# mnhrk15/integrated_path_planning

Measured on AMD Instinct MI355X. Metric: candidate trajectories/sec, higher is better.
Workload: dtype f64; 1 GPU; config4: 256 ego instances/GPU x 2240-candidate lattice (5 s, dt 0.1 s), 20-sample x 30-pedestrian x 51-step fp32 prediction distribution (layout [S][P][T][2]), eps=0; 8 distinct batches rotated (501 MB of obstacle tensors per GPU); instances_per_gpu=256, instances_total=256, rotation_batches=8, plan_calls_in_flight=4

## Files before the change

### integrated_path_planning_amd/csrc/fot_host.cpp

```cpp
#include <hip/hip_runtime.h>

#include <algorithm>
#include <cmath>
#include <cstddef>
#include <cstdlib>
#include <atomic>
#include <chrono>
#include <cstring>
#include <mutex>
#include <new>
#include <string>
#include <thread>
#include <unordered_set>
#include <vector>

#include "fot_kernels.h"
#include "fot_math.hpp"
#include "fot_replay.hpp"
#include "fot_summary.hpp"
#include "fot_loopscore.hpp"
#include "fot_setup.hpp"
#include "fot_sgan.h"

using namespace fot;
// ... 209 lines not shown
struct Scenario {
    fot_params params = fot_params();
    DevParams P;
    HostSpline spline;
    DevBuf dSpline;
    bool has_path = false;
    TileShapes shapes;
    int32_t shape_base = 0;
};

constexpr int FOT_LANES = 4;
constexpr int FOT_SPLIT_MIN_INSTANCES = 32;

struct fot_handle {
    int device = 0;
    hipStream_t stream = nullptr;
    hipEvent_t fork = nullptr;
    hipEvent_t order_done = nullptr;
    hipStream_t order_stream = nullptr;
    bool order_valid = false;
    int eval_segments = 0;
    PinnedBuf hDone;
    int32_t done_seq = 0;
    bool done_seq_armed = false;
    int tile_cut = 0;
    int eval_form = 0;
    int last_eval_forms = 0;
    std::vector<Scenario> sc;
    std::vector<ScenarioRef> refs;
    DevBuf dP;
    DevBuf dSplineTab;
    int32_t n_shape_entries = 0;
    DevBuf dShapes;
    Workspace ws[FOT_LANES];
    int lanes_cfg = 1;
    int lanes_used = 0;
    DevBuf dUserStatic, dUserDyn, dOut;
    PinnedBuf hSmallIn, hSmallOut;
    PinnedBuf hRecOut;
    PinnedBuf hScoreIn, hScoreOut;
    DevBuf dScoreT;
    DevBuf dTmpA, dTmpB, dTmpC, dTmpD;
    LoopState loop;
    struct Sgan {
        bool loaded = false;
        fot_sgan_desc desc{};
        SgDev dev{};
        DevBuf dImg, dOff, dScene, dObs, dNoise, dOut, dHenc, dPool, dCtx, dH, dC, dXY;
        PinnedBuf hTab;
        void release()
        {
            for (DevBuf *b : { &dImg, &dOff, &dScene, &dObs, &dNoise, &dOut, &dHenc, &dPool, &dCtx, &dH, &dC, &dXY }) b->release();
            hTab.release();
        }
    } sgan;
    bool last_valid = false;
    bool prof_on = false;
    std::vector<hipEvent_t> prof_pool;
    size_t prof_used = 0;
    std::vector<int> prof_kernel;
    int32_t prof_launches[FOT_PROFILE_KERNELS] = { 0 };
    double prof_ms[FOT_PROFILE_KERNELS] = { 0 };
    std::string err;
};

namespace {
// ... 96 lines not shown
int upload_params(fot_handle *h)
{
    std::vector<DevParams> tab(h->sc.size());
    for (size_t s = 0; s < h->sc.size(); ++s) tab[s] = h->sc[s].P;
    HIP_TRY(h, hipSetDevice(h->device));
    HIP_TRY(h, hipDeviceSynchronize());
    HIP_TRY(h, h->dP.ensure(sizeof(DevParams) * tab.size()));
    HIP_TRY(h, hipMemcpy(h->dP.p, tab.data(), sizeof(DevParams) * tab.size(), hipMemcpyHostToDevice));
    h->last_valid = false;
    return FOT_OK;
}

int upload_tile_shapes(fot_handle *h, int cut)
{
    const size_t n_sc = h->sc.size();
    std::vector<const DevParams *> ps(n_sc);
    std::vector<TileShapes> shapes(n_sc);
    for (size_t s = 0; s < n_sc; ++s) ps[s] = &h->sc[s].P;
    build_tile_shapes(ps.data(), (int)n_sc, shapes.data(), cut);
    std::vector<int32_t> cand0, nn, span;
    for (size_t s = 0; s < n_sc; ++s) {
        h->sc[s].shape_base = (int32_t)cand0.size();
        cand0.insert(cand0.end(), shapes[s].cand0.begin(), shapes[s].cand0.end());
        nn.insert(nn.end(), shapes[s].n.begin(), shapes[s].n.end());
        span.insert(span.end(), shapes[s].span.begin(), shapes[s].span.end());
        h->sc[s].shapes = std::move(shapes[s]);
    }
    h->refs.assign(n_sc, ScenarioRef());
    for (size_t s = 0; s < n_sc; ++s) {
        h->refs[s].hp = &h->sc[s].params; h->refs[s].P = &h->sc[s].P;
        h->refs[s].shapes = &h->sc[s].shapes; h->refs[s].shape_base = h->sc[s].shape_base;
    }
    h->tile_cut = cut;
    const size_t nt = cand0.size();
    h->n_shape_entries = (int32_t)nt;
    HIP_TRY(h, hipSetDevice(h->device));
    HIP_TRY(h, hipDeviceSynchronize());
    HIP_TRY(h, h->dShapes.ensure(sizeof(int32_t) * 3 * std::max<size_t>(nt, 1)));
    if (nt) {
        HIP_TRY(h, hipMemcpy(h->dShapes.p, cand0.data(), sizeof(int32_t) * nt, hipMemcpyHostToDevice));
        HIP_TRY(h, hipMemcpy(h->dShapes.as<int32_t>() + nt, nn.data(), sizeof(int32_t) * nt, hipMemcpyHostToDevice));
        HIP_TRY(h, hipMemcpy(h->dShapes.as<int32_t>() + 2 * nt, span.data(), sizeof(int32_t) * nt, hipMemcpyHostToDevice));
    }
    h->last_valid = false;
    return FOT_OK;
}

int check_scenarios(fot_handle *h, const fot_batch &b, const int32_t *scen)
{
    const int n_inst = b.n_inst;
    if (!scen) return h->sc[0].has_path ? FOT_OK : fail(h, FOT_ERR_NO_PATH_SET, "fot_set_path_* has not been called");
    for (int i = 0; i < n_inst; ++i) {
        if (scen[i] < 0 || scen[i] >= (int)h->sc.size()) return fail(h, FOT_ERR_INVALID, "unknown scenario id");
        if (!h->sc[(size_t)scen[i]].has_path)
            return fail(h, FOT_ERR_NO_PATH_SET, "an instance's scenario has no path (fot_set_scenario_path_*)");
    }
    for (int i = 1; i < n_inst && b.ego; ++i)
        if (b.ego[i].has_prev_s == FOT_PREV_S_CHAINED && scen[i] != scen[i - 1])
            return fail(h, FOT_ERR_INVALID, "a chained instance must be on its predecessor's scenario (a chain is one planner)");
    return FOT_OK;
    return FOT_OK;
}

PathSet path_set(const fot_handle *h, const BatchLayout &L, const DevParams **P_launch)
{
    const DevParams *dP = h->dP.as<DevParams>();
    if (L.scens.size() <= 1) {
        const int s = L.scens.empty() ? 0 : L.scens[0];
        *P_launch = dP + s;
        return PathSet::single(spline_view(h, s));
    }
    PathSet ps;
    ps.table = h->dSplineTab.as<SplineView>();
    ps.mixed = 1;
    for (int s : L.scens) ps.knots[ps.n_knots++] = h->sc[(size_t)s].spline.n;
// ... 65 lines not shown
    const size_t slots = (size_t)std::max<int64_t>(L.n_slots, 1);
    HIP_TRY(h, w.dCost.ensure(sizeof(double) * slots));
    HIP_TRY(h, w.dParts.ensure(sizeof(TilePart) * (size_t)std::max(L.n_tiles, 1)));
    HIP_TRY(h, w.dStatus.ensure(slots));
    HIP_TRY(h, w.dKeep.ensure(sizeof(uint16_t) * slots));
    const size_t n_ent = (size_t)L.n_entries + 64;
    HIP_TRY(h, w.dEntCnt.ensure(sizeof(int32_t) * (size_t)P.n_total * (size_t)L.n_inst));
    HIP_TRY(h, w.dEnt32.ensure(sizeof(f2) * n_ent));
    HIP_TRY(h, w.dEnt64.ensure(sizeof(d2) * n_ent));
    HIP_TRY(h, w.dEntSid.ensure(n_ent));
    HIP_TRY(h, w.dWaveRng.ensure(sizeof(TileStep) * (size_t)P.n_total * (size_t)std::max(L.n_tiles, 1)));
    HIP_TRY(h, w.dNanFlag.ensure((size_t)std::max<int64_t>(L.n_tracks, 16)));
    HIP_TRY(h, w.dDone.ensure(sizeof(int32_t) * (size_t)L.n_inst));

    w.staging_pending[slot] = true;

    const InstDesc *d_desc = (const InstDesc *)w.dMeta.p;
    TileTable tt;
    tt.cand0 = h->dShapes.as<int32_t>();
    tt.n = h->dShapes.as<int32_t>() + h->n_shape_entries;
    tt.span = h->dShapes.as<int32_t>() + 2 * (size_t)h->n_shape_entries;
    tt.n_tiles = L.n_tiles; tt.max_tiles = L.max_tiles; tt.row_budget = L.row_budget;
    tt.eval_segments = h->eval_segments;
    tt.grouped = L.grouped;
    tt.lean = h->eval_form == 0 ? 1 : 0;
    for (const Scenario &S : h->sc) if (S.P.n_total > WAVE || S.P.has_footprint) tt.lean = 0;
    for (int i = 0; i < L.n_inst && tt.lean; ++i) if (L.desc[(size_t)i].max_viol != 0) tt.lean = 0;
    h->last_eval_forms |= tt.lean ? 2 : 1;
    GroupHeadOut gh;
    if (evaluate_in_groups(tt)) {
        gh.n_pos = L.max_tiles / GROUP_TILES;
        HIP_TRY(h, w.dHeads.ensure(sizeof(GroupHead) * (size_t)L.n_inst * (size_t)gh.n_pos));
        gh.heads = tt.heads = w.dHeads.as<GroupHead>();
        gh.tile_cand0 = tt.cand0; gh.tile_n = tt.n;
    }
    const DevParams *dP = nullptr;
    const PathSet sv = path_set(h, L, &dP);
    CandArrays ca;
    ca.cost = w.dCost.as<double>(); ca.parts = w.dParts.as<TilePart>();
    ca.status = w.dStatus.as<uint8_t>(); ca.keep = w.dKeep.as<uint16_t>();
    if (sync_caller && h->done_seq_armed) { ca.done_flag = (int32_t *)h->hDone.p; ca.done_seq = h->done_seq; }

    EntryArrays ea;
    ea.cnt = w.dEntCnt.as<int32_t>(); ea.e32 = w.dEnt32.as<f2>(); ea.e64 = w.dEnt64.as<d2>();
    ea.sid = w.dEntSid.as<uint8_t>(); ea.rng = w.dWaveRng.as<TileStep>();
    ea.nan_flag = w.dNanFlag.as<uint8_t>();
    MetaImport imp;
    imp.h_desc = (const InstDesc *)stg;
    imp.d_desc = (InstDesc *)w.dMeta.p;
    static const bool eager_env = getenv("FOT_NAN_SCAN") && !std::strcmp(getenv("FOT_NAN_SCAN"), "eager");
    const bool eager_nan = eager_env || d_dyn_stage != nullptr;
    ea.eager_nan = eager_nan ? 1 : 0;
    NanScan scan;
    scan.eager = ea.eager_nan;
    if (L.n_tracks > 0 && (L.any_tmajor || eager_nan)) {
        scan.dyn_xy = d_dyn; scan.dtype = b.obstacle_dtype; scan.flag = w.dNanFlag.as<uint8_t>();
        scan.blocks_per_inst = (int)std::min<int64_t>(64, std::max<int64_t>(1, (L.max_dyn_bytes + 262143) / 262144));
        if (d_dyn_stage) {
            scan.stage = d_dyn_stage; d_dyn = d_dyn_stage;
            scan.blocks_per_inst = (int)std::min<int64_t>(64, std::max<int64_t>(1, (L.max_dyn_bytes + 65535) / 65536));
        }
    }
    {
        ProfScope ps(h, 0, st);
        LAUNCH_TRY(h, launch_frenet_state(dP, sv, d_desc, w.dState.as<InstState>(), L.n_inst, imp, scan, w.dDone.as<int32_t>(), st, gh));
    }
    if (L.any_obstacles) {
// ... 206 lines not shown
    return (int32_t)live_handles().size();
}

void fot_destroy(fot_handle *h)
{
    if (!h) return;
    {
        std::lock_guard<std::mutex> lk(g_live_mu);
        auto &live = live_handles();
        auto it = live.find(h);
        if (it == live.end()) return;
        live.erase(it);
    }
    destroy_handle(h);
}

}

namespace {

void destroy_handle(fot_handle *h)
{
    const double budget = destroy_timeout_s();
    bool quiet = hipSetDevice(h->device) == hipSuccess;
    if (quiet && h->stream) quiet = drained([&] { return hipStreamQuery(h->stream); }, budget);
    if (quiet && h->order_valid) quiet = drained([&] { return hipEventQuery(h->order_done); }, budget);
    for (Workspace &w : h->ws) if (quiet && w.stream) quiet = drained([&] { return hipStreamQuery(w.stream); }, budget);
    if (!quiet) {
        (void)hipGetLastError();
        delete h;
        return;
    }
    for (Scenario &S : h->sc) S.dSpline.release();
    DevBuf *bufs[] = { &h->dP, &h->dSplineTab, &h->dShapes, &h->dUserStatic, &h->dUserDyn, &h->dOut, &h->dTmpA, &h->dTmpB, &h->dTmpC, &h->dTmpD
                     };
    for (DevBuf *b : bufs) b->release();
    for (Workspace &w : h->ws) w.release();
    h->hSmallIn.release(); h->hSmallOut.release(); h->hRecOut.release(); h->hDone.release();
    h->hScoreIn.release(); h->hScoreOut.release(); h->dScoreT.release();
    h->sgan.release();
    h->loop.release();
    for (hipEvent_t e : h->prof_pool) (void)hipEventDestroy(e);
    if (h->fork) (void)hipEventDestroy(h->fork);
    if (h->order_done) (void)hipEventDestroy(h->order_done);
    if (h->stream) (void)hipStreamDestroy(h->stream);
    delete h;
}

}

extern "C" {

int fot_set_scenario_path_waypoints(fot_handle *h, int32_t id, int32_t n, const double *wx, const double *wy)
{
    if (!h) return FOT_ERR_INVALID;
    if (id < 0 || id >= (int)h->sc.size()) return fail(h, FOT_ERR_INVALID, "unknown scenario id");
    std::string err;
    HostSpline sp;
    int rc = build_spline(n, wx, wy, sp, err);
    if (rc != FOT_OK) return fail(h, rc, err);
    h->sc[(size_t)id].spline = sp;
    return upload_spline(h, id);
}

int fot_set_path_waypoints(fot_handle *h, int32_t n, const double *wx, const double *wy)
{
    return fot_set_scenario_path_waypoints(h, 0, n, wx, wy);
// ... 2535 lines not shown
```

### integrated_path_planning_amd/csrc/fot_kernels.h

```cpp
#pragma once

#include <cstddef>
#include <hip/hip_runtime.h>
#include "fot_types.h"
#include "fot_summary.hpp"
#include "fot_predscore.hpp"
#include "fot_loopscore.hpp"
#include "fot_repsample.hpp"

namespace fot {

struct TilePart {
    double cost;
    int32_t idx, keep;
    int32_t cnt[8];
};

struct CandArrays {
    double *cost;
    uint8_t *status;
    uint16_t *keep;
    TilePart *parts;
    int32_t *done_flag = nullptr;
    int32_t done_seq = 0;
// ... 12 lines not shown
    uint8_t *sid;
    TileStep *rng;
    const uint8_t *nan_flag = nullptr;
    int eager_nan = 0;
};

struct NanScan {
    const void *dyn_xy = nullptr;
    int dtype = 0;
    uint8_t *flag = nullptr;
    int blocks_per_inst = 0;
    int eager = 0;
    void *stage = nullptr;
};

struct MetaImport {
    const InstDesc *h_desc = nullptr;
    InstDesc *d_desc = nullptr;
};

struct TileTable {
    const int32_t *cand0 = nullptr, *n = nullptr;
    const int32_t *span = nullptr;
    int n_tiles = 0, max_tiles = 0, row_budget = 0;
    int grouped = 0;
    int eval_segments = 0;
    int lean = 0;
    GroupHead *heads = nullptr;
};
bool evaluate_in_groups(const TileTable &tiles);

struct GroupHeadOut {
    GroupHead *heads = nullptr;
    const int32_t *tile_cand0 = nullptr, *tile_n = nullptr;
    int n_pos = 0;
};

struct PathSet {
    SplineView one = SplineView();
    const SplineView *table = nullptr;
    int mixed = 0;
    int n_knots = 0;
    int knots[FOT_MAX_SCENARIOS] = { 0 };
    int fit_knots(int cap) const
    {
        int m = 0;
        for (int i = 0; i < n_knots; ++i) if (knots[i] <= cap && knots[i] > m) m = knots[i];
        return m;
    }
    static PathSet single(const SplineView &sp)
    {
        PathSet ps;
        ps.one = sp; ps.n_knots = 1; ps.knots[0] = sp.n;
        return ps;
    }
};

int launch_frenet_state(const DevParams *P, const PathSet &ps, const InstDesc *desc, InstState *state, int n_inst,
                        MetaImport imp, NanScan scan, int32_t *inst_done, hipStream_t st,
                        GroupHeadOut gh = GroupHeadOut());
int launch_cull(const DevParams *P, const InstDesc *desc, const InstState *state, int n_inst, int n_total, int n_ext,
                const PathSet &ps, const void *static_xy, const void *dyn_xy, int dtype, EntryArrays e, TileTable tiles,
                hipStream_t st);
int launch_evaluate(const DevParams *P, const PathSet &ps, const InstDesc *desc, const InstState *state, int n_total,
                    int n_inst, TileTable tiles, EntryArrays e, CandArrays c, fot_result *out, int32_t *inst_done,
                    hipStream_t st);
int launch_debug_path(const DevParams *P, const InstDesc *desc, const InstState *state,
// ... 94 lines not shown
```

### integrated_path_planning_amd/csrc/fot_kernels.hip

```cpp
#include <hip/hip_runtime.h>

#include <cstdlib>

#include "fot_math.hpp"
#include "fot_kernels.h"
#include "fot_summary.hpp"
#include "fot_predscore.hpp"
#include "fot_loopscore.hpp"
#include "fot_repsample.hpp"

namespace fot {


template <int CTRL, int ROW_MASK>
__device__ __forceinline__ float dpp_f32(float v)
{
    return __int_as_float(__builtin_amdgcn_update_dpp(__float_as_int(v), __float_as_int(v), CTRL, ROW_MASK, 0xf, false));
}

#define FOT_WAVE_REDUCE_F32(NAME, OP)                                                        \
    __device__ __forceinline__ float NAME(float v)                                           \
    {                                                                                        \
        v = OP(v, dpp_f32<0xB1, 0xf>(v));                           \
        v = OP(v, dpp_f32<0x4E, 0xf>(v));                           \
// ... 259 lines not shown
            const bool at_upper = fabs(best_s - s_max) < 1e-3 && s_max < s_end;
            need_global = at_lower || at_upper;
        }
        if (need_global) {
            ScanBest b = block_argmin(scan_samples(sp, x, y, 0.0, s_end, n_glob, tid, FRENET_WG, true), s_best);
            best_s = linspace_at(0.0, s_end, n_glob, b.idx >= 0 ? b.idx : 0);
        }
        if (!given) best_s = refine_nearest_wave(sp, x, y, best_s, lane);
        const double new_prev_s = given ? NAN : best_s;

        double fr[6], ref[6];
        bool ok = given ? frenet_state_given(sp, D.ego, fr, ref) : frenet_state_at(sp, D.ego, best_s, fr, ref);
        if (!ok && !given) {
            double px, py;
            spline_xy(sp, best_s, px, py);
            if (isnan(px) || isnan(py)) {
                ScanBest b = block_argmin(scan_samples(sp, x, y, 0.0, s_end, n_glob, tid, FRENET_WG, true), s_best);
                best_s = linspace_at(0.0, s_end, n_glob, b.idx >= 0 ? b.idx : 0);
                ok = frenet_state_at(sp, D.ego, best_s, fr, ref);
            }
        }
        const int nb = (ok && fr[1] > 0.1) ? P.n_brake : 0;
        const int n_cand = ok ? D.n_grid + nb : 0;
        if (tid == 0) {
            if (inst_done) inst_done[inst] = 0;
            InstState &S = state[inst];
            for (int i = 0; i < 6; ++i) { S.frenet0[i] = ok ? fr[i] : NAN; S.ref0[i] = ok ? ref[i] : NAN; }
            S.new_prev_s = new_prev_s;
            S.c2f_ok = ok ? 1 : 0;
            S.n_brake = nb;
            S.n_cand = n_cand;
        }
        if (gh.heads) {
            for (int t = tid; t < gh.n_pos * GROUP_MAX_PROFILES; t += FRENET_WG) {
                const int pos = t / GROUP_MAX_PROFILES, p = t - pos * GROUP_MAX_PROFILES;
                GroupHead &H = gh.heads[(int64_t)inst * gh.n_pos + pos];
                GroupStage G;
                const int32_t kind = group_head_stage(P, D, fr, ok ? 1 : 0, n_cand, gh.tile_cand0, gh.tile_n, pos, G);
                if (kind != GROUP_HEAD_FULL) {
                    if (p == 0) group_head_none(kind, G, H);
                    continue;
                }
                if (p == 0) group_head_common(P, D, fr, G, H);
                if (p < GROUP_TILES) group_head_tile(P, D, fr, n_cand, gh.tile_cand0, gh.tile_n, G, p, H);
                group_head_profile(P, D, fr, G, p, H);
            }
        }
        carry_prev_s = new_prev_s;
        chained = true;
    }
}

__global__ void __launch_bounds__(FRENET_WG)
k_frenet_state(const DevParams *__restrict__ Pp, SplineView sp_hbm, const SplineView *__restrict__ sp_table, int mixed,
               int lds_knots, const InstDesc *desc, InstState *__restrict__ state, int n_inst, MetaImport imp,
               NanScan scan, int32_t *__restrict__ inst_done, GroupHeadOut gh)
{
    SplineView sp = sp_hbm;
    if ((int)blockIdx.x < n_inst) {
        if (mixed) {
            const int scen = (imp.h_desc ? imp.h_desc : desc)[blockIdx.x].scen;
            Pp += scen;
            sp_hbm = load_const(sp_table, scen);
        }
        sp = stage_spline(sp_hbm, lds_knots);
    }
    frenet_state_block(Pp, sp, desc, state, n_inst, imp, scan, inst_done, (int)blockIdx.x, gh);
}


__device__ __forceinline__ double uniform_f64(double v)
{
    int lo = __builtin_amdgcn_readfirstlane(__double2loint(v));
    int hi = __builtin_amdgcn_readfirstlane(__double2hiint(v));
    asm volatile("" : "+s"(lo), "+s"(hi));
    return __hiloint2double(hi, lo);
}

// ... 2147 lines not shown
```

### integrated_path_planning_amd/csrc/fot_math.hpp

```cpp
#pragma once

#include <math.h>
#include "fot_types.h"

namespace fot {


FOT_HD double fast_rcp(double a)
{
#if defined(__HIP_DEVICE_COMPILE__)
    double x = __builtin_amdgcn_rcp(a);
    x = fma(x, fma(-a, x, 1.0), x);
#ifdef FOT_NEWTON2
    x = fma(x, fma(-a, x, 1.0), x);
#endif
    return x;
#else
    return 1.0 / a;
#endif
}

FOT_HD double fast_rsqrt(double a)
{
#if defined(__HIP_DEVICE_COMPILE__)
// ... 274 lines not shown
    sd = L.a1 + 2.0 * L.a2 * t + 3.0 * L.a3 * t2 + 4.0 * L.a4 * t3;
    sdd = 2.0 * L.a2 + 6.0 * L.a3 * t + 12.0 * L.a4 * t2;
    sddd = 6.0 * L.a3 + 24.0 * L.a4 * t;
}

FOT_HD void lat_eval(const double *q, double t, double &d, double &dd, double &ddd, double &dddd)
{
    const double b4 = FOT_FMA(t, q[5], q[4]);
    const double b3 = FOT_FMA(t, b4, q[3]);
    const double b2 = FOT_FMA(t, b3, q[2]);
    const double b1 = FOT_FMA(t, b2, q[1]);
    d = FOT_FMA(t, b1, q[0]);
    const double c4 = FOT_FMA(t, q[5], b4);
    const double c3 = FOT_FMA(t, c4, b3);
    const double c2 = FOT_FMA(t, c3, b2);
    dd = FOT_FMA(t, c2, b1);
    const double e4 = FOT_FMA(t, q[5], c4);
    const double e3 = FOT_FMA(t, e4, c3);
    ddd = 2.0 * FOT_FMA(t, e3, c2);
    dddd = 6.0 * q[3] + t * (24.0 * q[4] + t * (60.0 * q[5]));
}

FOT_HD void lon_sample(const LonInfo &L, int k, double dt, double &s, double &sd, double &sdd, double &sddd)
{
    if (k < L.n_eval) {
        lon_eval(L, (double)k * dt, s, sd, sdd, sddd);
    } else {
        double u0, u1, u2;
        lon_eval(L, (double)(L.n_eval - 1) * dt, s, u0, u1, u2);
        sd = 0.0; sdd = 0.0; sddd = 0.0;
    }
}

FOT_HD LonInfo profile_info(const DevParams &P, const InstDesc &D, const double *fr, int slot, bool with_summary)
{
    LonInfo L;
    const int n_grid_lon = P.n_ti * D.n_tv;
    if (slot < n_grid_lon) {
        const int ti = slot / D.n_tv, itv = slot - ti * D.n_tv;
        lon_coeffs(fr, tv_value(P, D, itv), P.ti[ti], L);
        L.n_t = P.ti[ti].n_t;
        L.n_eval = L.n_t;
    } else {
        const TimeInfo &tb = P.brake[slot - n_grid_lon];
        lon_coeffs(fr, 0.0, tb, L);
        L.n_t = P.n_total;
        L.n_eval = tb.n_t;
    }
    L.Js = 0.0; L.sd_last = 0.0;
    if (with_summary) {
#if defined(__clang__)
#pragma clang fp contract(off)
#endif
        const double n = (double)L.n_eval, c0 = 6.0 * L.a3, c1 = 24.0 * L.a4 * P.dt;
        const double sum_k = n * (n - 1.0) * 0.5, sum_k2 = (n - 1.0) * n * (2.0 * n - 1.0) / 6.0;
        L.Js = n * c0 * c0 + 2.0 * c0 * c1 * sum_k + c1 * c1 * sum_k2;
        if (L.n_t - 1 < L.n_eval) {
            const double t = (double)(L.n_t - 1) * P.dt, t2 = t * t, t3 = t2 * t;
            L.sd_last = L.a1 + 2.0 * L.a2 * t + 3.0 * L.a3 * t2 + 4.0 * L.a4 * t3;
        } else {
            L.sd_last = 0.0;
        }
    }
    return L;
}


FOT_HD int profile_rows(const DevParams &P, const InstDesc &D, int slot)
{
    const int n_grid_lon = P.n_ti * D.n_tv;
    if (slot < n_grid_lon) return P.ti[slot / D.n_tv].n_t;
    const int ne = P.brake[slot - n_grid_lon].n_t;
    return ne < P.n_total ? ne + 1 : ne;
}

#ifndef FOT_GROUP_TILES
#define FOT_GROUP_TILES 4
#endif
constexpr int GROUP_TILES = FOT_GROUP_TILES, GROUP_ROWS = 128 * FOT_GROUP_TILES, GROUP_MAX_PROFILES = 4 * FOT_GROUP_TILES;
FOT_HD int tile_row_budget(int n_total)
{
    const int want = 3 * n_total + 8, cap = 176;
    return want < cap ? want : (cap > n_total ? cap : n_total);
}

FOT_HD int tile_extent(const DevParams &P, const InstDesc &D, int cand0, int row_budget)
{
    const int n_grid_lon = P.n_ti * D.n_tv;
    int n = 0, rows = 0, profs = 0, c = cand0;
    while (n < WAVE && c < D.n_cand_max && profs < TILE_MAX_PROFILES) {
        int slot, left;
        if (c < D.n_grid) { slot = c / P.n_di; left = (slot + 1) * P.n_di - c; }
        else { slot = n_grid_lon + (c - D.n_grid); left = 1; }
        const int r = profile_rows(P, D, slot);
        if (profs > 0 && rows + r > row_budget) break;
        rows += r; ++profs;
        const int take = left < WAVE - n ? left : WAVE - n;
// ... 853 lines not shown
    H.ego_x = D.ego.x; H.ego_y = D.ego.y;
    for (int i = 0; i < 6; ++i) H.frenet0[i] = fr[i];
}

FOT_HD void group_head_tile(const DevParams &P, const InstDesc &D, const double *fr, int n_cand,
                            const int32_t *tile_cand0, const int32_t *tile_n, const GroupStage &G, int t, GroupHead &H)
{
    const int cand0 = tile_cand0[D.shape_off + G.grp_tile0 + t];
    int n = tile_n[D.shape_off + G.grp_tile0 + t];
    if (cand0 + n > n_cand) n = n_cand - cand0 > 0 ? n_cand - cand0 : 0;
    int own_lo = 0, own_hi = -1, n_loop = 0;
    if (n > 0) {
        own_lo = decode_candidate(P, D, fr, cand0).lon_slot - G.slot_lo;
        own_hi = decode_candidate(P, D, fr, cand0 + n - 1).lon_slot - G.slot_lo;
        for (int p = own_lo; p <= own_hi; ++p) {
            const int nt = profile_info(P, D, fr, G.slot_lo + p, false).n_t;
            n_loop = nt > n_loop ? nt : n_loop;
        }
    }
    H.t_cand0[t] = cand0; H.t_n[t] = n; H.t_n_loop[t] = n_loop; H.t_own_lo[t] = own_lo; H.t_own_hi[t] = own_hi;
}

FOT_HD void group_head_profile(const DevParams &P, const InstDesc &D, const double *fr, const GroupStage &G, int p,
                               GroupHead &H)
{
    LonInfo L;
    if (p < G.n_stage) {
        L = profile_info(P, D, fr, G.slot_lo + p, true);
    } else {
        L.a0 = L.a1 = L.a2 = L.a3 = L.a4 = L.Js = L.sd_last = L.T = 0.0;
        L.n_t = 0; L.n_eval = 0;
    }
    H.info[p] = L;
}

FOT_HD void build_group_head(const DevParams &P, const InstDesc &D, const double *fr, int c2f_ok, int n_cand,
                             const int32_t *tile_cand0, const int32_t *tile_n, int pos, GroupHead &H)
{
    GroupStage G;
    const int32_t kind = group_head_stage(P, D, fr, c2f_ok, n_cand, tile_cand0, tile_n, pos, G);
    if (kind != GROUP_HEAD_FULL) { group_head_none(kind, G, H); return; }
    group_head_common(P, D, fr, G, H);
    for (int t = 0; t < GROUP_TILES; ++t) group_head_tile(P, D, fr, n_cand, tile_cand0, tile_n, G, t, H);
    for (int p = 0; p < GROUP_MAX_PROFILES; ++p) group_head_profile(P, D, fr, G, p, H);
}

#if defined(__HIP_DEVICE_COMPILE__)
__device__ __attribute__((noinline))
#else
inline
#endif
double yaw_from_sin_cos(double sn, double cs) { return atan2(sn, cs); }

template <class Tab>
FOT_HD void final_sample(const DevParams &P, const LonInfo &L, const Tab &lon_tab, const double *q, int k,
                         double *o )
{
    double s, sd, sdd, sddd, d, d_d, d_dd, d_ddd;
    lon_sample(L, k, P.dt, s, sd, sdd, sddd);
    lat_sample(q, k, L.n_eval, P.dt, d, d_d, d_dd, d_ddd);
    LonSample ls;
    lon_tab.load(k, ls);
    CartSample c;
    frenet_to_cart(ls, d, d_d, d_dd, c);
    o[0] = (double)k * P.dt;
    o[1] = ls.s; o[2] = ls.sd; o[3] = ls.sdd; o[4] = sddd;
// ... 129 lines not shown
```

### integrated_path_planning_amd/csrc/fot_setup.hpp

```cpp
#pragma once

#include <cmath>
#include <string>
#include <cstdlib>
#include <vector>

#include "fot_types.h"
#include "fot_math.hpp"

namespace fot {


inline bool time_info(double T, double dt, TimeInfo &ti)
{
    ti.T = T;
    ti.n_t = (int)std::nearbyint(T / dt) + 1;
    if (ti.n_t < 1 || ti.n_t > FOT_MAX_NT) return false;
    const double T2 = T * T, T3 = T2 * T, T4 = T2 * T2, T5 = T4 * T;
    {
        const double a = 3.0 * T2, b = 4.0 * T3, c = 6.0 * T, d = 12.0 * T2;
        const double det = a * d - b * c;
        ti.qa[0] = d / det; ti.qa[1] = -b / det; ti.qa[2] = -c / det; ti.qa[3] = a / det;
    }
    {
        const double m[3][3] = { { T3, T4, T5 }, { 3.0 * T2, 4.0 * T3, 5.0 * T4 }, { 6.0 * T, 12.0 * T2, 20.0 * T3 } };
        double cof[3][3];
        for (int r = 0; r < 3; ++r)
            for (int c = 0; c < 3; ++c) {
                const int r1 = (r + 1) % 3, r2 = (r + 2) % 3, c1 = (c + 1) % 3, c2 = (c + 2) % 3;
                cof[r][c] = m[r1][c1] * m[r2][c2] - m[r1][c2] * m[r2][c1];
            }
        const double det = m[0][0] * cof[0][0] + m[0][1] * cof[0][1] + m[0][2] * cof[0][2];
        for (int r = 0; r < 3; ++r)
            for (int c = 0; c < 3; ++c) ti.qi[r * 3 + c] = cof[c][r] / det;
    }
// ... 195 lines not shown
            if (T.n[(size_t)t] <= 0) continue;
            int s0, s1;
            wave_profile_span(P, D, P.n_ti * n_tv, T.cand0[(size_t)t], T.cand0[(size_t)t] + T.n[(size_t)t] - 1, s0, s1);
            T.span[(size_t)t] = (int32_t)(((uint32_t)s0 << 16) | (uint32_t)s1);
        }
    }
}

enum { TILE_CUT_AUTO = 0, TILE_CUT_WAVE = 1, TILE_CUT_GROUP = 2 };
inline void build_tile_shapes(const DevParams *const *P, int n, TileShapes *T, int cut = TILE_CUT_AUTO)
{
    std::vector<TileShapes> wave((size_t)n), grouped((size_t)n);
    int64_t n_wave = 0, n_grouped = 0;
    for (int s = 0; s < n; ++s) {
        build_tile_shapes_wave(*P[s], wave[(size_t)s]);
        build_tile_shapes_grouped(*P[s], grouped[(size_t)s]);
        n_wave += wave[(size_t)s].n_real;
        n_grouped += grouped[(size_t)s].n_real;
    }
    bool use_groups = (double)n_grouped <= 1.15 * (double)n_wave;
    if (cut == TILE_CUT_WAVE) use_groups = false;
    if (cut == TILE_CUT_GROUP) use_groups = true;
    for (int s = 0; s < n; ++s) {
        T[s] = use_groups ? grouped[(size_t)s] : wave[(size_t)s];
        fill_tile_spans(*P[s], T[s]);
    }
}
inline void build_tile_shapes(const DevParams &P, TileShapes &T, int cut = TILE_CUT_AUTO)
{
    const DevParams *one = &P;
    build_tile_shapes(&one, 1, &T, cut);
}

struct BatchLayout {
    std::vector<InstDesc> desc;
    int n_inst = 0;
    int n_tiles = 0;
    int max_tiles = 0;
    int row_budget = 0;
    int grouped = 0;
    int64_t n_slots = 0;
    int64_t n_lon = 0;
    int max_lon = 0;
    int64_t n_static = 0;
    int64_t dyn_src_points = 0;
    int64_t n_entries = 0;
    int64_t n_tracks = 0;
    int64_t max_dyn_bytes = 0;
    bool any_obstacles = false;
    bool any_tmajor = false;
    int n_ext = 0;
    std::vector<int32_t> scens;
};

struct ScenarioRef {
    const fot_params *hp = nullptr;
    const DevParams *P = nullptr;
    const TileShapes *shapes = nullptr;
    int32_t shape_base = 0;
};

inline int build_batch_layout(const ScenarioRef *sc, int n_scen, const int32_t *scen, const fot_batch &b,
                              BatchLayout &L, std::string &err)
{
    L = BatchLayout();
    if (n_scen < 1 || !sc) { err = "no scenario"; return FOT_ERR_INVALID; }
    if (b.n_inst < 0) { err = "n_inst < 0"; return FOT_ERR_INVALID; }
    if (b.n_inst > 0 && (!b.ego || !b.target_speed)) { err = "ego / target_speed missing"; return FOT_ERR_INVALID; }
    if (b.obstacle_dtype != FOT_F32 && b.obstacle_dtype != FOT_F64) { err = "obstacle_dtype"; return FOT_ERR_INVALID; }
    L.n_inst = b.n_inst;
    L.desc.resize(b.n_inst);
    L.grouped = sc[0].shapes->grouped;
    for (int s = 0; s < n_scen; ++s)
        if (sc[s].shapes->row_budget > L.row_budget) L.row_budget = sc[s].shapes->row_budget;
    std::vector<uint8_t> used((size_t)n_scen, 0);
    for (int i = 0; i < b.n_inst; ++i) {
        InstDesc &D = L.desc[i];
        D = InstDesc();
        D.ego = b.ego[i];
        const int si = scen ? scen[i] : 0;
        if (si < 0 || si >= n_scen) { err = "unknown scenario id"; return FOT_ERR_INVALID; }
        const fot_params &hp = *sc[si].hp;
        const DevParams &P = *sc[si].P;
        const TileShapes &shapes = *sc[si].shapes;
        D.scen = si;
        used[(size_t)si] = 1;
        if (D.ego.has_prev_s < 0 || D.ego.has_prev_s > FOT_EGO_IS_FRENET) { err = "has_prev_s must be 0 .. 3"; return FOT_ERR_INVALID; }
        if (i == 0 && D.ego.has_prev_s == FOT_PREV_S_CHAINED) { err = "the first instance cannot be chained"; return FOT_ERR_INVALID; }
        if (i > 0 && D.ego.has_prev_s == FOT_PREV_S_CHAINED && si != L.desc[i - 1].scen) {
            err = "a chained instance must be on its predecessor's scenario (a chain is one planner)"; return FOT_ERR_INVALID;
        }
        const double target = b.target_speed[i];
        D.target_speed = target;
// ... 106 lines not shown
```

### integrated_path_planning_amd/csrc/fot_types.h

```cpp
#pragma once

#include <stdint.h>
#include "../../include/fot.h"

#if defined(__HIPCC__) || defined(__HIP__)
#define FOT_HD __host__ __device__ __forceinline__
#else
#define FOT_HD inline
#endif

namespace fot {

constexpr int WAVE = 64;
constexpr int WAVES_PER_GROUP = 4;
constexpr int TILE_MAX_PROFILES = 8;
constexpr int N_XCD = 8;
constexpr int LON_FIELDS = 10;
constexpr int ST_PENDING = FOT_ST_OK;

struct d2 { double x, y; };
struct f2 { float x, y; };
constexpr float FAR32 = 1.0e18f;

struct TimeInfo {
    double T;
    double qa[4];
    double qi[9];
    int32_t n_t;
    int32_t _pad;
};

struct DevParams {
    double max_speed, max_accel, max_curvature, max_lat_accel;
    double dt, d_road_w, max_road_width, min_t, d_t_s;
// ... 61 lines not shown
    double sd_last;
    double T;
    int32_t n_t;
    int32_t n_eval;
};

constexpr int GROUP_HEAD_TILES = 4, GROUP_HEAD_PROFILES = 16;
enum : int32_t {
    GROUP_HEAD_ABSENT = 0,
    GROUP_HEAD_EMPTY = 2,
    GROUP_HEAD_FULL = 1
};
struct alignas(128) GroupHead {
    int32_t present;
    int32_t grp_tile0;
    int32_t slot_lo, n_stage;
    int32_t total_rows;
    int32_t n_total, n_circ_fp;
    int32_t cand_off, tile0, ent_cap, max_viol;
    int32_t n_grid, n_tv, n_di, n_side, n_ti;
    int32_t row0[GROUP_HEAD_PROFILES + 1];
    int32_t t_cand0[GROUP_HEAD_TILES], t_n[GROUP_HEAD_TILES];
    int32_t t_n_loop[GROUP_HEAD_TILES];
    int32_t t_own_lo[GROUP_HEAD_TILES], t_own_hi[GROUP_HEAD_TILES];
    int64_t ent_off;
    double d_road_w, dt, road_lim;
    double lim_speed, lim_accel, lim_curv, lim_lat;
    double ego_x, ego_y;
    double frenet0[6];
    LonInfo info[GROUP_HEAD_PROFILES];
};
static_assert(sizeof(GroupHead) % 128 == 0 && sizeof(GroupHead) == 1536, "whole 128-byte lines");

}
```

Baseline: 2.726 billion candidates/s.

## Precompute per-tile-group header templates at path setup and compose heads from them

Builds instance-independent GroupHead templates (tile staging, per-profile slot indices, n_t/n_eval) on the host once per tile-table change and uploads them. The frenet kernel's head-building loop then copies the template words, fills in the instance-specific fields, and recomputes only the per-profile longitudinal coefficients, replacing the per-instance group_head_stage, common, tile and profile logic. The aim is to cut per-plan work in the setup kernel, at the cost of a new device buffer and the assumption that template fields do not depend on the instance's state beyond the brake/grid variant and c2f_ok.

```diff
diff --git a/integrated_path_planning_amd/csrc/fot_host.cpp b/integrated_path_planning_amd/csrc/fot_host.cpp
--- a/integrated_path_planning_amd/csrc/fot_host.cpp
+++ b/integrated_path_planning_amd/csrc/fot_host.cpp
@@ -265,6 +265,8 @@
     DevBuf dSplineTab;
     int32_t n_shape_entries = 0;
     DevBuf dShapes;
+    int head_tmpl_entries = 0;
+    DevBuf dHeadTmpl;
     Workspace ws[FOT_LANES];
     int lanes_cfg = 1;
     int lanes_used = 0;
@@ -427,6 +429,10 @@
         h->refs[s].shapes = &h->sc[s].shapes; h->refs[s].shape_base = h->sc[s].shape_base;
     }
     h->tile_cut = cut;
+    std::vector<HeadTemplate> tmpl;
+    h->head_tmpl_entries = head_template_entries(h->refs.data(), (int)n_sc);
+    if (h->head_tmpl_entries > 0)
+        build_head_templates(h->refs.data(), (int)n_sc, cand0.data(), nn.data(), h->head_tmpl_entries, tmpl);
     const size_t nt = cand0.size();
     h->n_shape_entries = (int32_t)nt;
     HIP_TRY(h, hipSetDevice(h->device));
@@ -436,6 +442,10 @@
         HIP_TRY(h, hipMemcpy(h->dShapes.p, cand0.data(), sizeof(int32_t) * nt, hipMemcpyHostToDevice));
         HIP_TRY(h, hipMemcpy(h->dShapes.as<int32_t>() + nt, nn.data(), sizeof(int32_t) * nt, hipMemcpyHostToDevice));
         HIP_TRY(h, hipMemcpy(h->dShapes.as<int32_t>() + 2 * nt, span.data(), sizeof(int32_t) * nt, hipMemcpyHostToDevice));
+    }
+    if (!tmpl.empty()) {
+        HIP_TRY(h, h->dHeadTmpl.ensure(sizeof(HeadTemplate) * tmpl.size()));
+        HIP_TRY(h, hipMemcpy(h->dHeadTmpl.p, tmpl.data(), sizeof(HeadTemplate) * tmpl.size(), hipMemcpyHostToDevice));
     }
     h->last_valid = false;
     return FOT_OK;
@@ -567,7 +577,8 @@
         gh.n_pos = L.max_tiles / GROUP_TILES;
         HIP_TRY(h, w.dHeads.ensure(sizeof(GroupHead) * (size_t)L.n_inst * (size_t)gh.n_pos));
         gh.heads = tt.heads = w.dHeads.as<GroupHead>();
-        gh.tile_cand0 = tt.cand0; gh.tile_n = tt.n;
+        gh.tmpl = h->dHeadTmpl.as<HeadTemplate>(); gh.tmpl_entries = h->head_tmpl_entries;
+        if (gh.tmpl_entries < 1) return fail(h, FOT_ERR_INVALID, "plan: no header templates for this handle's tile table");
     }
     const DevParams *dP = nullptr;
     const PathSet sv = path_set(h, L, &dP);
@@ -840,7 +851,7 @@
         return;
     }
     for (Scenario &S : h->sc) S.dSpline.release();
-    DevBuf *bufs[] = { &h->dP, &h->dSplineTab, &h->dShapes, &h->dUserStatic, &h->dUserDyn, &h->dOut, &h->dTmpA, &h->dTmpB, &h->dTmpC, &h->dTmpD
+    DevBuf *bufs[] = { &h->dP, &h->dSplineTab, &h->dShapes, &h->dHeadTmpl, &h->dUserStatic, &h->dUserDyn, &h->dOut, &h->dTmpA, &h->dTmpB, &h->dTmpC, &h->dTmpD
                      };
     for (DevBuf *b : bufs) b->release();
     for (Workspace &w : h->ws) w.release();
diff --git a/integrated_path_planning_amd/csrc/fot_kernels.h b/integrated_path_planning_amd/csrc/fot_kernels.h
--- a/integrated_path_planning_amd/csrc/fot_kernels.h
+++ b/integrated_path_planning_amd/csrc/fot_kernels.h
@@ -68,7 +68,8 @@
 
 struct GroupHeadOut {
     GroupHead *heads = nullptr;
-    const int32_t *tile_cand0 = nullptr, *tile_n = nullptr;
+    const HeadTemplate *tmpl = nullptr;
+    int tmpl_entries = 0;
     int n_pos = 0;
 };
 
diff --git a/integrated_path_planning_amd/csrc/fot_kernels.hip b/integrated_path_planning_amd/csrc/fot_kernels.hip
--- a/integrated_path_planning_amd/csrc/fot_kernels.hip
+++ b/integrated_path_planning_amd/csrc/fot_kernels.hip
@@ -315,18 +315,11 @@
             S.n_cand = n_cand;
         }
         if (gh.heads) {
+            const int variant = nb > 0 ? HEAD_VARIANT_BRAKE : HEAD_VARIANT_GRID;
             for (int t = tid; t < gh.n_pos * GROUP_MAX_PROFILES; t += FRENET_WG) {
                 const int pos = t / GROUP_MAX_PROFILES, p = t - pos * GROUP_MAX_PROFILES;
-                GroupHead &H = gh.heads[(int64_t)inst * gh.n_pos + pos];
-                GroupStage G;
-                const int32_t kind = group_head_stage(P, D, fr, ok ? 1 : 0, n_cand, gh.tile_cand0, gh.tile_n, pos, G);
-                if (kind != GROUP_HEAD_FULL) {
-                    if (p == 0) group_head_none(kind, G, H);
-                    continue;
-                }
-                if (p == 0) group_head_common(P, D, fr, G, H);
-                if (p < GROUP_TILES) group_head_tile(P, D, fr, n_cand, gh.tile_cand0, gh.tile_n, G, p, H);
-                group_head_profile(P, D, fr, G, p, H);
+                group_head_compose(P, D, fr, ok ? 1 : 0, gh.tmpl[head_template_index(D, variant, gh.tmpl_entries, pos)], p,
+                                   gh.heads[(int64_t)inst * gh.n_pos + pos]);
             }
         }
         carry_prev_s = new_prev_s;
diff --git a/integrated_path_planning_amd/csrc/fot_math.hpp b/integrated_path_planning_amd/csrc/fot_math.hpp
--- a/integrated_path_planning_amd/csrc/fot_math.hpp
+++ b/integrated_path_planning_amd/csrc/fot_math.hpp
@@ -330,6 +330,22 @@
     }
 }
 
+FOT_HD void lon_summary(const DevParams &P, LonInfo &L)
+{
+#if defined(__clang__)
+#pragma clang fp contract(off)
+#endif
+    const double n = (double)L.n_eval, c0 = 6.0 * L.a3, c1 = 24.0 * L.a4 * P.dt;
+    const double sum_k = n * (n - 1.0) * 0.5, sum_k2 = (n - 1.0) * n * (2.0 * n - 1.0) / 6.0;
+    L.Js = n * c0 * c0 + 2.0 * c0 * c1 * sum_k + c1 * c1 * sum_k2;
+    if (L.n_t - 1 < L.n_eval) {
+        const double t = (double)(L.n_t - 1) * P.dt, t2 = t * t, t3 = t2 * t;
+        L.sd_last = L.a1 + 2.0 * L.a2 * t + 3.0 * L.a3 * t2 + 4.0 * L.a4 * t3;
+    } else {
+        L.sd_last = 0.0;
+    }
+}
+
 FOT_HD LonInfo profile_info(const DevParams &P, const InstDesc &D, const double *fr, int slot, bool with_summary)
 {
     LonInfo L;
@@ -346,21 +362,19 @@
         L.n_eval = tb.n_t;
     }
     L.Js = 0.0; L.sd_last = 0.0;
-    if (with_summary) {
-#if defined(__clang__)
-#pragma clang fp contract(off)
-#endif
-        const double n = (double)L.n_eval, c0 = 6.0 * L.a3, c1 = 24.0 * L.a4 * P.dt;
-        const double sum_k = n * (n - 1.0) * 0.5, sum_k2 = (n - 1.0) * n * (2.0 * n - 1.0) / 6.0;
-        L.Js = n * c0 * c0 + 2.0 * c0 * c1 * sum_k + c1 * c1 * sum_k2;
-        if (L.n_t - 1 < L.n_eval) {
-            const double t = (double)(L.n_t - 1) * P.dt, t2 = t * t, t3 = t2 * t;
-            L.sd_last = L.a1 + 2.0 * L.a2 * t + 3.0 * L.a3 * t2 + 4.0 * L.a4 * t3;
-        } else {
-            L.sd_last = 0.0;
-        }
-    }
+    if (with_summary) lon_summary(P, L);
     return L;
+}
+
+struct LonSlot { int ti, itv; };
+
+FOT_HD LonSlot lon_slot(const DevParams &P, const InstDesc &D, int slot)
+{
+    LonSlot s;
+    const int n_grid_lon = P.n_ti * D.n_tv;
+    if (slot < n_grid_lon) { s.ti = slot / D.n_tv; s.itv = slot - s.ti * D.n_tv; }
+    else { s.ti = slot - n_grid_lon; s.itv = -1; }
+    return s;
 }
 
 
@@ -1280,6 +1294,60 @@
         L.n_t = 0; L.n_eval = 0;
     }
     H.info[p] = L;
+}
+
+
+FOT_HD bool head_instance_dword(int w)
+{
+    return (w >= (int)offsetof(GroupHead, cand_off) / 4 && w < (int)offsetof(GroupHead, n_grid) / 4) ||
+           (w >= (int)offsetof(GroupHead, ent_off) / 4 && w < (int)offsetof(GroupHead, d_road_w) / 4) ||
+           (w >= (int)offsetof(GroupHead, lim_speed) / 4 && w < (int)offsetof(GroupHead, info) / 4);
+}
+
+FOT_HD void group_head_instance(const InstDesc &D, const double *fr, GroupHead &H)
+{
+    H.cand_off = D.cand_off; H.tile0 = D.tile0; H.ent_cap = D.ent_cap; H.max_viol = D.max_viol;
+    H.ent_off = D.ent_off;
+    H.lim_speed = D.lim_speed; H.lim_accel = D.lim_accel; H.lim_curv = D.lim_curv; H.lim_lat = D.lim_lat;
+    H.ego_x = D.ego.x; H.ego_y = D.ego.y;
+    for (int i = 0; i < 6; ++i) H.frenet0[i] = fr[i];
+}
+
+FOT_HD void group_head_profile_at(const DevParams &P, const InstDesc &D, const double *fr, const HeadProfile &hp, LonInfo &L)
+{
+    if (hp.n_t > 0) {
+        lon_coeffs(fr, hp.itv >= 0 ? tv_value(P, D, hp.itv) : 0.0, hp.itv >= 0 ? P.ti[hp.ti] : P.brake[hp.ti], L);
+        L.n_t = hp.n_t; L.n_eval = hp.n_eval;
+        lon_summary(P, L);
+    } else {
+        L.a0 = L.a1 = L.a2 = L.a3 = L.a4 = L.Js = L.sd_last = L.T = 0.0;
+        L.n_t = 0; L.n_eval = 0;
+    }
+}
+
+FOT_HD void group_head_compose(const DevParams &P, const InstDesc &D, const double *fr, int c2f_ok, const HeadTemplate &T,
+                               int p, GroupHead &H)
+{
+    int32_t kind = (int32_t)T.common[0];
+    if (!c2f_ok && kind == GROUP_HEAD_FULL) kind = GROUP_HEAD_EMPTY;
+    if (kind != GROUP_HEAD_FULL) {
+        if (p == 0) {
+            H.present = kind;
+            if (kind == GROUP_HEAD_EMPTY) H.grp_tile0 = (int32_t)T.common[1];
+        }
+        return;
+    }
+    uint32_t *dst = (uint32_t *)(void *)&H;
+    for (int w = p; w < HEAD_COMMON_DWORDS; w += GROUP_MAX_PROFILES)
+        if (!head_instance_dword(w)) dst[w] = T.common[w];
+    if (p == 0) group_head_instance(D, fr, H);
+    group_head_profile_at(P, D, fr, T.prof[p], H.info[p]);
+}
+
+FOT_HD int64_t head_template_index(const InstDesc &D, int variant, int n_entries, int pos)
+{
+    const int g = pos < D.n_tiles / GROUP_TILES ? D.shape_off / GROUP_TILES + pos : n_entries - 1;
+    return (int64_t)variant * n_entries + g;
 }
 
 FOT_HD void build_group_head(const DevParams &P, const InstDesc &D, const double *fr, int c2f_ok, int n_cand,
diff --git a/integrated_path_planning_amd/csrc/fot_setup.hpp b/integrated_path_planning_amd/csrc/fot_setup.hpp
--- a/integrated_path_planning_amd/csrc/fot_setup.hpp
+++ b/integrated_path_planning_amd/csrc/fot_setup.hpp
@@ -1,6 +1,8 @@
 #pragma once
 
+#include <algorithm>
 #include <cmath>
+#include <cstring>
 #include <string>
 #include <cstdlib>
 #include <vector>
@@ -262,6 +264,32 @@
     build_tile_shapes(&one, 1, &T, cut);
 }
 
+inline void build_head_template(const DevParams &P, const InstDesc &D, int n_cand, const int32_t *tile_cand0,
+                                const int32_t *tile_n, int pos, HeadTemplate &T)
+{
+    const double fr[6] = { 0.0, 0.0, 0.0, 0.0, 0.0, 0.0 };
+    GroupHead H;
+    std::memset((void *)&H, 0, sizeof H);
+    std::memset((void *)&T, 0, sizeof T);
+    GroupStage G = GroupStage();
+    const int32_t kind = group_head_stage(P, D, fr, 1, n_cand, tile_cand0, tile_n, pos, G);
+    if (kind != GROUP_HEAD_FULL) {
+        group_head_none(kind, G, H);
+    } else {
+        group_head_common(P, D, fr, G, H);
+        for (int t = 0; t < GROUP_TILES; ++t) group_head_tile(P, D, fr, n_cand, tile_cand0, tile_n, G, t, H);
+        for (int p = 0; p < G.n_stage; ++p) {
+            const LonSlot s = lon_slot(P, D, G.slot_lo + p);
+            const LonInfo L = profile_info(P, D, fr, G.slot_lo + p, false);
+            HeadProfile &hp = T.prof[p];
+            hp.ti = s.ti; hp.itv = s.itv; hp.n_t = L.n_t; hp.n_eval = L.n_eval; hp.T = L.T;
+        }
+    }
+    uint32_t words[HEAD_COMMON_DWORDS];
+    std::memcpy(words, &H, sizeof words);
+    for (int w = 0; w < HEAD_COMMON_DWORDS; ++w) T.common[w] = head_instance_dword(w) ? 0u : words[w];
+}
+
 struct BatchLayout {
     std::vector<InstDesc> desc;
     int n_inst = 0;
@@ -289,6 +317,34 @@
     const TileShapes *shapes = nullptr;
     int32_t shape_base = 0;
 };
+
+inline int head_template_entries(const ScenarioRef *sc, int n)
+{
+    int64_t tiles = 0;
+    for (int s = 0; s < n; ++s) {
+        if (!sc[s].shapes->grouped) return 0;
+        tiles += (int64_t)sc[s].shapes->cand0.size();
+    }
+    return (int)(tiles / GROUP_TILES) + 1;
+}
+
+inline void build_head_templates(const ScenarioRef *sc, int n, const int32_t *tile_cand0, const int32_t *tile_n, int n_entries,
+                                 std::vector<HeadTemplate> &out)
+{
+    out.assign((size_t)HEAD_VARIANTS * (size_t)n_entries, HeadTemplate());
+    for (int s = 0; s < n; ++s)
+        for (int n_tv = 1; n_tv <= FOT_MAX_TV; ++n_tv) {
+            const DevParams &P = *sc[s].P;
+            InstDesc D = shape_desc(P, n_tv);
+            D.scen = s;
+            D.shape_off = sc[s].shape_base + sc[s].shapes->off[n_tv];
+            D.n_tiles = sc[s].shapes->tiles_of(n_tv);
+            for (int v = 0; v < HEAD_VARIANTS; ++v)
+                for (int pos = 0; pos <= D.n_tiles / GROUP_TILES; ++pos)
+                    build_head_template(P, D, v == HEAD_VARIANT_BRAKE ? D.n_cand_max : D.n_grid, tile_cand0, tile_n, pos,
+                                        out[(size_t)head_template_index(D, v, n_entries, pos)]);
+        }
+}
 
 inline int build_batch_layout(const ScenarioRef *sc, int n_scen, const int32_t *scen, const fot_batch &b,
                               BatchLayout &L, std::string &err)
diff --git a/integrated_path_planning_amd/csrc/fot_types.h b/integrated_path_planning_amd/csrc/fot_types.h
--- a/integrated_path_planning_amd/csrc/fot_types.h
+++ b/integrated_path_planning_amd/csrc/fot_types.h
@@ -1,5 +1,6 @@
 #pragma once
 
+#include <stddef.h>
 #include <stdint.h>
 #include "../../include/fot.h"
 
@@ -127,4 +128,19 @@
 };
 static_assert(sizeof(GroupHead) % 128 == 0 && sizeof(GroupHead) == 1536, "whole 128-byte lines");
 
+constexpr int HEAD_COMMON_DWORDS = 344 / 4;
+enum : int32_t { HEAD_VARIANT_GRID = 0, HEAD_VARIANT_BRAKE = 1, HEAD_VARIANTS = 2 };
+struct HeadProfile {
+    int32_t ti, itv;
+    int32_t n_t, n_eval;
+    double T;
+};
+struct alignas(128) HeadTemplate {
+    uint32_t common[HEAD_COMMON_DWORDS];
+    uint32_t _pad[2];
+    HeadProfile prof[GROUP_HEAD_PROFILES];
+};
+static_assert(sizeof(HeadTemplate) == 768, "whole 128-byte lines");
+static_assert(offsetof(GroupHead, info) == 4 * HEAD_COMMON_DWORDS, "HeadTemplate::common is the GroupHead in front of info");
+
 }
```

Measured after the change: 2.755 billion candidates/s (median of 6 runs). 1.01x the previous value.
